# worldfnd/provekit

Hardware: AMD Instinct MI355X
Metric: proofs/sec (noir-r1cs prove hot path, WHIR commit + sumcheck + folding rounds) (higher is better)
Workload: dtype u32x8 (BN254-Fr, 256-bit Montgomery integers); 1 GPU; poseidon-rounds size class: m=21, m_0=20, satisfiable synthetic R1CS (786429 constraints, 1048571 witnesses, a constant term in half of the rows of A and B), batch-2 WHIR commit + zk-sumcheck + 4-round WHIR opening, queries [109, 28, 16, 11]/9, pow_bits [19.0, 16.0, 16.0, 18.0]/11.0 (WhirConfig::new derivation, security 128, ConjectureList), blinding WHIR n=8 queries [122]/31, Skyscraper-sponge tr; launcher=single process

## Files before the change

provekit_amd/csrc/ntt.hip:

```cpp
#include <algorithm>
#include <map>
#include <mutex>
#include <vector>

#include <atomic>

#define PK_BASE_PRIO 1
#include "internal.hpp"
#include "ntt_regs.hpp"

using namespace pk;

namespace {

constexpr int BT = 4;
constexpr int NTHREADS = 256;

__device__ __forceinline__ fe root28_mont() {
    fe r;
    r.v[0] = 0x725b19f0u; r.v[1] = 0x9bd61b6eu; r.v[2] = 0x41112ed4u; r.v[3] = 0x402d111eu;
    r.v[4] = 0x8ef62abcu; r.v[5] = 0x00e0a7ebu; r.v[6] = 0xa58a7e85u; r.v[7] = 0x2a3c09f0u;
    return fe_to_montx(r);
}

__global__ void twiddle_init_kernel(fe* W, unsigned log_n) {
    if (threadIdx.x == 0 && blockIdx.x == 0) {
        fe_store(W, fe_one());
        fe w = root28_mont();
        for (unsigned i = log_n; i < 28; i++) w = fe_sqrx(w);
        if (log_n > 0) fe_store(W + 1, w);
    }
}
__global__ __launch_bounds__(256) void twiddle_double_kernel(fe* W, size_t h) {
    size_t j = (size_t)blockIdx.x * blockDim.x + threadIdx.x;
    if (j >= h) return;
    fe wh = fe_load(W + h);
    if (j == 0) return;
    fe_store(W + h + j, fe_mulx(fe_load(W + j), wh));
}
__global__ void twiddle_seed_kernel(fe* W, size_t h) {
    if (threadIdx.x == 0 && blockIdx.x == 0) fe_store(W + h, fe_sqrx(fe_load(W + h / 2)));
}

__global__ __launch_bounds__(256) void twiddle_scale_kernel(const fe* __restrict__ W, fe* __restrict__ Ws, size_t n) {
    size_t j = (size_t)blockIdx.x * blockDim.x + threadIdx.x;
    if (j >= n) return;
    fe c = fe_zero();
    c.v[0] = 32u;
    fe_store(Ws + j, fe_mulx(fe_load(W + j), c));
}

__global__ __launch_bounds__(256) void twiddle_shoup_kernel(const fe* __restrict__ X, u32* __restrict__ T, size_t n) {
    size_t j = (size_t)blockIdx.x * blockDim.x + threadIdx.x;
    if (j >= n) return;
    const fe29 c = unpack29<0>(fe_from_montx(fe_load(X + j)));
    const fe29 cq = shoup_quotient29(c);
#pragma unroll
    for (int l = 0; l < 9; l++) T[TW29S_WORDS * j + l] = c.v[l];
#pragma unroll
    for (int l = 0; l < 9; l++) T[TW29S_WORDS * j + 9 + l] = cq.v[l];
}

__global__ __launch_bounds__(256) void twiddle_pass_table_kernel(const u32* __restrict__ src, u32* __restrict__ T, size_t rows_k, size_t row, size_t mul,
                                                                 size_t mask) {
    const size_t i = (size_t)blockIdx.x * blockDim.x + threadIdx.x;
    if (i >= rows_k * row) return;
    const size_t k = i / row, v = i % row;
    const u32* q = src + TW29S_WORDS * ((mul * k * v) & mask);
#pragma unroll
    for (int l = 0; l < TW29S_WORDS; l++) T[TW29S_WORDS * i + l] = q[l];
}

struct PassParams {
    const fe* in;
    fe* out;
    size_t in_col_stride, out_col_stride;
    size_t in_stride_r, in_stride_v, in_stride_u;
    size_t out_stride_r, out_stride_v, out_stride_u;
    unsigned log_v;
    size_t nonzero;
    size_t in_nat_r, in_nat_v, in_nat_u;
    const fe* W;
    const fe* Wtw;
    const u32* W29;
    const u32* Wtw29;
    const u32* Tpass29;
    size_t tp_row;
    size_t tiles;
    unsigned ncols;
    int xcd_tiles;
    int lazy_store;
    size_t n_mask;
    size_t tw_mul;
    size_t wr_step;
    const fe* in_poly[16];
    unsigned in_fold;
    int pre_terms;
    size_t pre_stride, pre_elem, pre_ku, pre_kv;
    const u32* Wpre29;
};

template <int LOG_R, bool IN_R_CONTIG>
__global__ __launch_bounds__(NTHREADS) void ntt_pass_kernel(PassParams p) {
    PK_LATENCY_PRIO();
    constexpr int R = 1 << LOG_R;
    constexpr int TILE = R * BT;
    extern __shared__ uint4 lds[];
    uint4* lo = lds;
    uint4* hi = lds + TILE;
    uint4* wlo = lds + 2 * TILE;
    uint4* whi = wlo + (R / 2 > 0 ? R / 2 : 1);

    const unsigned tid = threadIdx.x;
    const size_t tile = blockIdx.x;
    const size_t vblocks = ((size_t)1 << p.log_v) / BT;
    const size_t u = tile / vblocks, vb = tile % vblocks;
    const size_t v0 = vb * BT;
    const size_t col = blockIdx.y;
    const fe* in = p.in + col * p.in_col_stride + u * p.in_stride_u + v0 * p.in_stride_v;
    fe* out = p.out + col * p.out_col_stride + u * p.out_stride_u + v0 * p.out_stride_v;
    const size_t nat0 = u * p.in_nat_u + v0 * p.in_nat_v;

    for (int j = tid; j < R / 2; j += NTHREADS) {
        const uint4* q = reinterpret_cast<const uint4*>(p.W + (size_t)j * p.wr_step);
        wlo[j] = q[0];
        whi[j] = q[1];
    }
    for (int e = tid; e < TILE; e += NTHREADS) {
        int r, b;
        if (IN_R_CONTIG) {
            r = e % R;
            b = e / R;
        } else {
            b = e % BT;
            r = e / BT;
        }
        size_t nat = nat0 + (size_t)r * p.in_nat_r + (size_t)b * p.in_nat_v;
        uint4 a0 = make_uint4(0, 0, 0, 0), a1 = a0;
        if (nat < p.nonzero) {
            const uint4* q = reinterpret_cast<const uint4*>(in + (size_t)r * p.in_stride_r + (size_t)b * p.in_stride_v);
            a0 = q[0];
            a1 = q[1];
        }
        lo[r * BT + b] = a0;
        hi[r * BT + b] = a1;
    }
    __syncthreads();

#pragma unroll 1
    for (int s = 0; s < LOG_R; s++) {
        const int half = R >> (s + 1);
        for (int t = tid; t < (R / 2) * BT; t += NTHREADS) {
            int b = t % BT, j = t / BT;
            int pos = j & (half - 1);
            int i0 = ((j - pos) << 1) + pos;
            int i1 = i0 + half;
            int a0i = i0 * BT + b, a1i = i1 * BT + b;
            fe x0, x1;
            {
                uint4 l0 = lo[a0i], h0 = hi[a0i], l1 = lo[a1i], h1 = hi[a1i];
                x0.v[0] = l0.x; x0.v[1] = l0.y; x0.v[2] = l0.z; x0.v[3] = l0.w;
                x0.v[4] = h0.x; x0.v[5] = h0.y; x0.v[6] = h0.z; x0.v[7] = h0.w;
                x1.v[0] = l1.x; x1.v[1] = l1.y; x1.v[2] = l1.z; x1.v[3] = l1.w;
                x1.v[4] = h1.x; x1.v[5] = h1.y; x1.v[6] = h1.z; x1.v[7] = h1.w;
            }
            fe sum = fe_add(x0, x1);
            fe dif = fe_sub(x0, x1);
            int widx = pos << s;
            if (widx != 0) {
                uint4 wl = wlo[widx], wh = whi[widx];
                fe w;
                w.v[0] = wl.x; w.v[1] = wl.y; w.v[2] = wl.z; w.v[3] = wl.w;
                w.v[4] = wh.x; w.v[5] = wh.y; w.v[6] = wh.z; w.v[7] = wh.w;
                dif = fe_mulx(dif, w);
            }
            lo[a0i] = make_uint4(sum.v[0], sum.v[1], sum.v[2], sum.v[3]);
            hi[a0i] = make_uint4(sum.v[4], sum.v[5], sum.v[6], sum.v[7]);
            lo[a1i] = make_uint4(dif.v[0], dif.v[1], dif.v[2], dif.v[3]);
            hi[a1i] = make_uint4(dif.v[4], dif.v[5], dif.v[6], dif.v[7]);
        }
        __syncthreads();
    }

    for (int e = tid; e < TILE; e += NTHREADS) {
        int b = e % BT, k = e / BT;
        int r = LOG_R == 0 ? 0 : (int)(__brev((unsigned)k) >> (LOG_R ? 32 - LOG_R : 1));
        uint4 l0 = lo[r * BT + b], h0 = hi[r * BT + b];
        fe x;
        x.v[0] = l0.x; x.v[1] = l0.y; x.v[2] = l0.z; x.v[3] = l0.w;
        x.v[4] = h0.x; x.v[5] = h0.y; x.v[6] = h0.z; x.v[7] = h0.w;
        if (p.tw_mul != 0) {
            size_t ex = (p.tw_mul * (size_t)k * (v0 + b)) & p.n_mask;
            if (ex != 0) x = fe_mulx(x, fe_load(p.W + ex));
        }
        fe_store(out + (size_t)k * p.out_stride_r + (size_t)b * p.out_stride_v, x);
    }
}

__host__ __device__ __forceinline__ constexpr int bitrev_c(int v, int bits) {
    int r = 0;
    for (int i = 0; i < bits; i++) r |= ((v >> i) & 1) << (bits - 1 - i);
    return r;
}

struct Ntt8Ctx {
    const fe* in;
    const fe* cin;
    fe* out;
    size_t nat0, v0, k10;
    unsigned tid;
};

template <int LE, int LOG_R, int J, bool PRE>
__device__ __forceinline__ void ntt8_round(fe29 (&x)[1 << LE], const PassParams& p, const Ntt8Ctx& c, u32* planes) {
    constexpr int NX = 1 << LE;
    constexpr int LOGB = 11 - LOG_R, BTT = 1 << LOGB;
    constexpr int NR = (LOG_R + LE - 1) / LE;
    constexpr int D0 = LOG_R - LE * (NR - 1);
    constexpr int D = J == 0 ? D0 : LE;
    constexpr int DONE = J == 0 ? 0 : D0 + LE * (J - 1);
    constexpr int POS = LOGB + LOG_R - DONE - D;
    constexpr int E = LE - D;
    constexpr int REST = POS - LOGB;
    constexpr int LO = POS - E;
    const unsigned tid = c.tid;
    const int base_idx = (int)((tid & ((1u << LO) - 1)) << E) | (int)((tid >> LO) << (POS + D));
#define PK_TILE_INDEX(reg) (base_idx | ((reg) & ((1 << E) - 1)) | (((reg) >> E) << POS))
    if (J == 0) {
#pragma unroll
        for (int reg = 0; reg < NX; reg++) {
            const int I = PK_TILE_INDEX(reg);
            const int r = I >> LOGB, b = I & (BTT - 1);
            const size_t nat = c.nat0 + (size_t)r * p.in_nat_r + (size_t)b * p.in_nat_v;
            if constexpr (PRE) {
                const size_t k1 = c.k10 + (size_t)b * p.pre_kv;
                x[reg] = pre_load_sum(p.pre_terms, [&](int n1, fe29& y) {
                    const size_t t = nat + (size_t)n1 * p.pre_stride;
                    if (t >= p.nonzero) return false;
                    y = mul_tw(unpack29<0>(fe_load(c.cin + t * p.pre_elem)), tw29s_load(p.Wpre29, (k1 * t) & p.n_mask));
                    return true;
                });
            } else {
                fe t = fe_zero();
                if (nat < p.nonzero) t = fe_load(c.in + (size_t)r * p.in_stride_r + (size_t)b * p.in_stride_v);
                x[reg] = unpack29<0>(t);
            }
        }
    } else {
        __syncthreads();
#pragma unroll
        for (int reg = 0; reg < NX; reg++) {
            const int I = PK_TILE_INDEX(reg);
#pragma unroll
            for (int l = 0; l < 9; l++) x[reg].v[l] = planes[l * 2048 + I];
        }
        __syncthreads();
    }
    dft_regs<LE, D>(x);
    const int m = (base_idx >> LOGB) & ((1 << REST) - 1);
    if (J + 1 < NR) {
        const size_t unit = p.wr_step << (LOG_R - D - REST);
#pragma unroll
        for (int reg = 0; reg < NX; reg++) {
            const int a = bitrev_c(reg >> E, D);
            fe29 y = a == 0 ? red29(x[reg]) : mul_tw(x[reg], tw29s_load(p.W29, (size_t)(a * m) * unit));
            const int I = (PK_TILE_INDEX(reg) & ~(((1 << D) - 1) << POS)) | (a << POS);
#pragma unroll
            for (int l = 0; l < 9; l++) planes[l * 2048 + I] = y.v[l];
        }
    } else {
        const int rr = base_idx >> LOGB;
        int k_hi = 0;
#pragma unroll
        for (int j = 0; j < J; j++) {
            const int dj = j == 0 ? D0 : LE, done_j = j == 0 ? 0 : D0 + LE * (j - 1);
            k_hi |= ((rr >> (LOG_R - done_j - dj)) & ((1 << dj) - 1)) << done_j;
        }
        constexpr int KLO = DONE;
#pragma unroll
        for (int reg = 0; reg < NX; reg++) {
            const int a = bitrev_c(reg >> E, D);
            const int b = PK_TILE_INDEX(reg) & (BTT - 1);
            const int k = k_hi | (a << KLO);
            fe29 y;
            if (p.tw_mul && p.Tpass29) {
                y = mul_tw(x[reg], tw29s_load(p.Tpass29, (size_t)k * p.tp_row + (c.v0 + b)));
            } else if (p.tw_mul) {
                size_t ex = (p.tw_mul * (size_t)k * (c.v0 + b)) & p.n_mask;
                y = mul_tw(x[reg], tw29s_load(p.Wtw29, ex));
            } else {
                y = a == 0 ? red29(x[reg]) : red29w(x[reg]);
            }
            fe_store(c.out + (size_t)k * p.out_stride_r + (size_t)b * p.out_stride_v, p.lazy_store ? pack29(y) : pack_canon29(y));
        }
    }
#undef PK_TILE_INDEX
}

template <int LE, int LOG_R, int J, bool PRE>
__device__ __forceinline__ void ntt8_rounds_from(fe29 (&x)[1 << LE], const PassParams& p, const Ntt8Ctx& c, u32* planes) {
    constexpr int NR = (LOG_R + LE - 1) / LE;
    if constexpr (J < NR) {
        ntt8_round<LE, LOG_R, J, PRE>(x, p, c, planes);
        ntt8_rounds_from<LE, LOG_R, J + 1, PRE>(x, p, c, planes);
    }
}

template <int LE, int LOG_R, bool IN_R_CONTIG, bool PRE>
__global__ __launch_bounds__(2048 >> LE) __attribute__((amdgpu_waves_per_eu(4, 4))) void ntt8_pass_kernel(PassParams p) {
    PK_LATENCY_PRIO();
    constexpr int LOGB = 11 - LOG_R;
    extern __shared__ u32 planes[];
    const size_t vblocks = ((size_t)1 << p.log_v) >> LOGB;
    size_t tile, col;
    if (p.xcd_tiles) {
        const size_t j = blockIdx.x >> 3;
        col = j % p.ncols;
        tile = (j / p.ncols) * 8 + (blockIdx.x & 7);
    } else {
        tile = blockIdx.x % p.tiles;
        col = blockIdx.x / p.tiles;
    }
    const size_t u = tile / vblocks, vb = tile % vblocks;
    Ntt8Ctx c;
    c.v0 = vb << LOGB;
    c.cin = p.in_poly[0] ? p.in_poly[col >> p.in_fold] + (col & (((size_t)1 << p.in_fold) - 1)) : p.in + col * p.in_col_stride;
    c.in = c.cin + u * p.in_stride_u + c.v0 * p.in_stride_v;
    c.k10 = u * p.pre_ku + c.v0 * p.pre_kv;
    c.out = p.out + col * p.out_col_stride + u * p.out_stride_u + c.v0 * p.out_stride_v;
    c.nat0 = u * p.in_nat_u + c.v0 * p.in_nat_v;
    c.tid = threadIdx.x;
    fe29 x[1 << LE];
    ntt8_rounds_from<LE, LOG_R, 0, PRE>(x, p, c, planes);
}

template <int FW_MAX>
__global__ __launch_bounds__(256) void deinterleave_kernel(const fe* __restrict__ c, fe* __restrict__ S, size_t L, unsigned fw,
                                                           size_t col_stride) {
    PK_LATENCY_PRIO();
    extern __shared__ uint4 tl[];
    const unsigned TT = 1024 / fw;
    size_t t0 = (size_t)blockIdx.x * TT;
    const fe* src = c + t0 * fw;
    for (unsigned e = threadIdx.x; e < 1024; e += 256) {
        size_t t = t0 + e / fw;
        uint4 a0 = make_uint4(0, 0, 0, 0), a1 = a0;
        if (t < L) {
            const uint4* q = reinterpret_cast<const uint4*>(src + e);
            a0 = q[0];
            a1 = q[1];
        }
        tl[2 * e] = a0;
        tl[2 * e + 1] = a1;
    }
    __syncthreads();
    for (unsigned e = threadIdx.x; e < 1024; e += 256) {
        unsigned j = e / TT, tt = e % TT;
        size_t t = t0 + tt;
        if (t < L) {
            unsigned src_e = tt * fw + j;
            uint4* q = reinterpret_cast<uint4*>(S + (size_t)j * col_stride + t);
            q[0] = tl[2 * src_e];
            q[1] = tl[2 * src_e + 1];
        }
    }
}

__global__ __launch_bounds__(256) void ntt_shard_prestep_kernel(const fe* __restrict__ S, size_t s_col_stride, size_t L, fe* __restrict__ Y,
                                                                size_t y_col_stride, size_t Ng , unsigned g, unsigned G,
                                                                const fe* __restrict__ W , size_t n_mask) {
    PK_LATENCY_PRIO();
    const size_t col = blockIdx.y;
    const fe* x = S + col * s_col_stride;
    fe* y = Y + col * y_col_stride;
    const size_t stride = (size_t)gridDim.x * blockDim.x;
    for (size_t n = (size_t)blockIdx.x * blockDim.x + threadIdx.x; n < Ng; n += stride) {
        fe acc = fe_zero();
        for (unsigned s = 0; s < G; s++) {
            size_t idx = n + (size_t)s * Ng;
            if (idx >= L) break;
            fe v = fe_load(x + idx);
            size_t e = ((size_t)((s * g) % G) * Ng) & n_mask;
            if (e) v = fe_mulx(v, fe_load(W + e));
            acc = fe_add(acc, v);
        }
        size_t e = (n * (size_t)g) & n_mask;
        if (e) acc = fe_mulx(acc, fe_load(W + e));
        fe_store(y + n, acc);
    }
}

struct TableStore {
    std::mutex mu;
    std::map<unsigned long long, void*> tables;
    unsigned contexts = 0;
};
TableStore& store_of(int device) {
    static std::mutex mu;
    static std::map<int, TableStore> stores;
    std::lock_guard<std::mutex> lock(mu);
    return stores[device];
}
enum TableKind : unsigned long long { TK_W = 1, TK_WS = 2, TK_W29 = 3, TK_WS29 = 4, TK_PASS = 5 };
template <class T, class Fill>
int table(pk_ctx* ctx, TableKind kind, unsigned key, size_t bytes, const T** out, Fill fill) {
    const unsigned long long id = (kind << 56) | key;
    auto it = ctx->tables.find(id);
    if (it == ctx->tables.end()) {
        TableStore& S = store_of(ctx->device);
        std::lock_guard<std::mutex> lock(S.mu);
        auto st = S.tables.find(id);
        if (st == S.tables.end()) {
            T* made = nullptr;
            PK_HIP(ctx, hipMalloc((void**)&made, bytes));
            fill(made);
            PK_LAUNCH_CHECK(ctx);
            PK_WAIT(ctx);
            st = S.tables.emplace(id, (void*)made).first;
        }
        it = ctx->tables.emplace(id, st->second).first;
    }
    *out = (const T*)it->second;
    return PK_OK;
}

int get_twiddles(pk_ctx* ctx, unsigned log_n, const fe** out) {
    const size_t n = (size_t)1 << log_n;
    return table(ctx, TK_W, log_n, 32 * std::max<size_t>(n, 2), out, [&](fe* W) {
        twiddle_init_kernel<<<1, 64, 0, ctx->stream>>>(W, log_n);
        for (size_t h = 2; h < n; h <<= 1) {
            twiddle_seed_kernel<<<1, 64, 0, ctx->stream>>>(W, h);
            unsigned grid = (unsigned)((h + 255) / 256);
            twiddle_double_kernel<<<grid, 256, 0, ctx->stream>>>(W, h);
        }
    });
}

struct Twiddles {
    const fe *W, *Ws;
    const u32 *W29, *Ws29;
};
int get_tables(pk_ctx* ctx, unsigned log_n, bool scaled, Twiddles* t) {
    const size_t n = (size_t)1 << log_n, entries = std::max<size_t>(n, 2);
    const unsigned grid = (unsigned)((n + 255) / 256);
    *t = Twiddles{};
    int rc = get_twiddles(ctx, log_n, &t->W);
    t->Ws = t->W;
    if (!rc && scaled)
        rc = table(ctx, TK_WS, log_n, 32 * entries, &t->Ws, [&](fe* Ws) { twiddle_scale_kernel<<<grid, 256, 0, ctx->stream>>>(t->W, Ws, n); });
    if (rc || log_n < 3) return rc;
    auto shoup = [&](TableKind kind, const fe* X, const u32** out) {
        return table(ctx, kind, log_n, 4 * TW29S_WORDS * entries, out, [&](u32* U) { twiddle_shoup_kernel<<<grid, 256, 0, ctx->stream>>>(X, U, n); });
    };
    rc = shoup(TK_W29, t->W, &t->W29);
    t->Ws29 = t->W29;
    if (!rc && scaled) rc = shoup(TK_WS29, t->Ws, &t->Ws29);
    return rc;
}

inline bool pass_is_fast(unsigned log_r, unsigned log_v, size_t N) { return log_r >= 3 && log_v < 62 && log_v >= 11 - log_r && N >= 8; }

constexpr int NTT_LE = 2;

int set_lds_once(pk_ctx* ctx, const void* kernel, size_t lds_bytes, std::atomic<unsigned long long>& done) {
    const unsigned long long dev_bit = 1ull << (ctx->device & 63);
    if (!(done.load(std::memory_order_acquire) & dev_bit)) {
        PK_HIP(ctx, hipFuncSetAttribute(kernel, hipFuncAttributeMaxDynamicSharedMemorySize, (int)lds_bytes));
        done.fetch_or(dev_bit, std::memory_order_release);
    }
    return PK_OK;
}

template <int LE, int LOG_R, bool CONTIG, bool PRE>
int launch_fast(pk_ctx* ctx, const PassParams& pp, unsigned grid) {
    const size_t lds_bytes = 9 * 2048 * 4;
    static std::atomic<unsigned long long> lds_set{0};
    if (int rc = set_lds_once(ctx, (const void*)ntt8_pass_kernel<LE, LOG_R, CONTIG, PRE>, lds_bytes, lds_set)) return rc;
    ntt8_pass_kernel<LE, LOG_R, CONTIG, PRE><<<dim3(grid, 1), 2048 >> LE, lds_bytes, ctx->stream>>>(pp);
    PK_LAUNCH_CHECK(ctx);
    return PK_OK;
}

template <int LOG_R, bool CONTIG>
int launch_lds(pk_ctx* ctx, const PassParams& p, dim3 grid) {
    constexpr int R = 1 << LOG_R;
    const size_t lds_bytes = (size_t)(2 * R * BT + 2 * (R / 2 > 0 ? R / 2 : 1)) * 16;
    static std::atomic<unsigned long long> lds_set{0};
    if (int rc = set_lds_once(ctx, (const void*)ntt_pass_kernel<LOG_R, CONTIG>, lds_bytes, lds_set)) return rc;
    ntt_pass_kernel<LOG_R, CONTIG><<<grid, NTHREADS, lds_bytes, ctx->stream>>>(p);
    PK_LAUNCH_CHECK(ctx);
    return PK_OK;
}

template <int LOG_R>
int launch_pass_r(pk_ctx* ctx, const PassParams& p, bool in_r_contig, size_t tiles, unsigned ncols) {
    if (pass_is_fast(LOG_R, p.log_v, p.n_mask + 1)) {
        ProfScope prof(ctx, in_r_contig ? "ntt_pass_last" : "ntt_pass");
        const size_t tiles8 = (tiles * BT) >> (11 - LOG_R);
        PassParams pp = p;
        pp.tiles = tiles8;
        pp.ncols = ncols;
        pp.xcd_tiles = ((p.Tpass29 != nullptr || p.in_poly[0] != nullptr) && tiles8 % 8 == 0) ? 1 : 0;
        PK_REQUIRE(ctx, tiles8 * ncols < ((size_t)1 << 31), "NTT launch too large");
        const unsigned grid = (unsigned)(tiles8 * ncols);
        constexpr int LR = LOG_R >= 3 ? LOG_R : 3;
        if (p.pre_terms)
            return in_r_contig ? launch_fast<NTT_LE, LR, true, true>(ctx, pp, grid) : launch_fast<NTT_LE, LR, false, true>(ctx, pp, grid);
        return in_r_contig ? launch_fast<NTT_LE, LR, true, false>(ctx, pp, grid) : launch_fast<NTT_LE, LR, false, false>(ctx, pp, grid);
    }
    PK_REQUIRE(ctx, p.in_poly[0] == nullptr && p.pre_terms == 0, "fused NTT input needs the register-radix pass");
    ProfScope prof(ctx, in_r_contig ? "ntt_pass_last" : "ntt_pass");
    const dim3 grid((unsigned)tiles, ncols);
    return in_r_contig ? launch_lds<LOG_R, true>(ctx, p, grid) : launch_lds<LOG_R, false>(ctx, p, grid);
}

int launch_pass(pk_ctx* ctx, unsigned log_r, const PassParams& p, bool in_r_contig, size_t tiles, unsigned ncols) {
    switch (log_r) {
        case 0: return launch_pass_r<0>(ctx, p, in_r_contig, tiles, ncols);
        case 1: return launch_pass_r<1>(ctx, p, in_r_contig, tiles, ncols);
        case 2: return launch_pass_r<2>(ctx, p, in_r_contig, tiles, ncols);
        case 3: return launch_pass_r<3>(ctx, p, in_r_contig, tiles, ncols);
        case 4: return launch_pass_r<4>(ctx, p, in_r_contig, tiles, ncols);
        case 5: return launch_pass_r<5>(ctx, p, in_r_contig, tiles, ncols);
        case 6: return launch_pass_r<6>(ctx, p, in_r_contig, tiles, ncols);
        case 7: return launch_pass_r<7>(ctx, p, in_r_contig, tiles, ncols);
        case 8: return launch_pass_r<8>(ctx, p, in_r_contig, tiles, ncols);
        case 9: return launch_pass_r<9>(ctx, p, in_r_contig, tiles, ncols);
    }
    return set_err(ctx, PK_ERR_BAD_ARG, "unsupported radix 2^%u", log_r);
}

}

namespace pk {

void ntt_retain_ctx(pk_ctx* ctx) {
    TableStore& S = store_of(ctx->device);
    std::lock_guard<std::mutex> lock(S.mu);
    S.contexts++;
}
void ntt_release_ctx(pk_ctx* ctx) {
    ctx->tables.clear();
    TableStore& S = store_of(ctx->device);
    std::lock_guard<std::mutex> lock(S.mu);
    if (S.contexts && --S.contexts == 0) {
        for (auto& kv : S.tables) (void)hipFree(kv.second);
        S.tables.clear();
    }
}

constexpr size_t PRE_MAX_TERMS = 3;
static_assert(PRE_MAX_TERMS <= 4, "pre_load_sum: red29 takes a sum of at most four products");

struct NttPlan {
    unsigned P;
    unsigned l[3];
    unsigned log_v[3];
    bool fast[3];
    size_t L1;
    bool pre;
};
NttPlan ntt_plan(unsigned log_n, size_t nonzero) {
    NttPlan q{};
    const size_t N = (size_t)1 << log_n;
    q.P = log_n <= 18 ? 2 : 3;
    unsigned left = log_n;
    for (unsigned i = 0; i < q.P; i++) {
        q.l[i] = (left + q.P - i - 1) / (q.P - i);
        left -= q.l[i];
        q.log_v[i] = i + 1 < q.P ? left : q.l[0];
        q.fast[i] = pass_is_fast(q.l[i], q.log_v[i], N);
    }
    const size_t stride1 = N >> q.l[0];
    q.L1 = std::max<size_t>(1, (std::min(nonzero, N) + stride1 - 1) / stride1);
    q.pre = q.L1 <= PRE_MAX_TERMS && q.fast[1];
    return q;
}

bool ntt_scaled_available(unsigned log_n) {
    if (log_n <= 9 || log_n > 27) return false;
    const NttPlan q = ntt_plan(log_n, 0);
    return q.fast[q.P - 2];
}

bool ntt_reads_polys(unsigned log_n, size_t nonzero) {
    if (log_n <= 9) return false;
    const NttPlan q = ntt_plan(log_n, nonzero);
    return q.pre || q.fast[0];
}

struct NttInput {
    const fe* in;
    size_t col_stride;
    const fe* const* polys;
    unsigned fold, npolys;
};

struct NttRun {
    NttPlan plan;
    unsigned log_n;
    bool scaled_out;
    Twiddles tw;
    NttInput src;
    size_t nonzero;
    size_t e;
    fe* scratch;
    fe* out;
    size_t out_col_stride;
};

constexpr unsigned PASS_TABLE_MIN_LOG_N = 19;

static int pass_params(pk_ctx* ctx, const NttRun& t, unsigned i, PassParams* out) {
    const NttPlan& q = t.plan;
    const bool last = i + 1 == q.P;
    const size_t N = (size_t)1 << t.log_n, R1 = (size_t)1 << q.l[0], S1 = N / R1;
    unsigned done = 0;
    for (unsigned j = 0; j < i; j++) done += q.l[j];
    const size_t K = (size_t)1 << done, R = (size_t)1 << q.l[i], S = N / (K * R);
    auto tw29 = [&](unsigned j) { return j + 2 == q.P ? t.tw.Ws29 : t.tw.W29; };
    PassParams p{};
    p.W = t.tw.W;
    p.W29 = t.tw.W29;
    p.Wtw = i + 2 == q.P ? t.tw.Ws : t.tw.W;
    p.Wtw29 = tw29(i);
    p.n_mask = N - 1;
    p.log_v = q.log_v[i];
    p.wr_step = N >> q.l[i];
    if (!last) {
        p.out = t.scratch;
        p.out_col_stride = N;
        p.out_stride_r = S;
        p.out_stride_v = 1;
        p.out_stride_u = i ? R * S : 0;
        p.tw_mul = K;
        p.tp_row = S;
        p.lazy_store = q.fast[i + 1];
    } else {
        p.out = t.out;
        p.out_col_stride = t.out_col_stride;
        p.out_stride_r = K;
        p.out_stride_v = 1;
        p.out_stride_u = q.P == 3 ? R1 : 0;
        p.lazy_store = t.scaled_out;
    }
    if (i == 0 || (i == 1 && q.pre)) {
        p.in = t.src.in;
        p.in_col_stride = t.src.col_stride;
        if (t.src.polys) {
            for (unsigned b = 0; b < t.src.npolys; b++) p.in_poly[b] = t.src.polys[b];
            p.in_fold = t.src.fold;
        }
        p.nonzero = t.nonzero;
        p.in_nat_r = S;
        p.in_nat_v = last ? 0 : 1;
        if (i == 0) {
            p.in_stride_r = S * t.e;
            p.in_stride_v = t.e;
        } else {
            p.pre_terms = (int)q.L1;
            p.pre_stride = S1;
            p.pre_elem = t.e;
            p.pre_ku = last ? 0 : 1;
            p.pre_kv = last ? 1 : 0;
            p.Wpre29 = tw29(0);
        }
    } else {
        p.in = t.scratch;
        p.in_col_stride = N;
        p.nonzero = 1;
        p.in_stride_r = last ? 1 : S;
        p.in_stride_v = last ? S1 : 1;
        p.in_stride_u = last ? (q.P == 3 ? R : 0) : R * S;
    }
    if (!last && t.log_n >= PASS_TABLE_MIN_LOG_N && q.fast[i]) {
        const unsigned key = t.log_n | ((i + 1) << 8) | ((t.scaled_out && i + 2 == q.P ? 1u : 0u) << 12);
        const u32* src = p.Wtw29;
        int rc = table(ctx, TK_PASS, key, 4 * TW29S_WORDS * R * S, &p.Tpass29, [&](u32* T) {
            twiddle_pass_table_kernel<<<(unsigned)((R * S + 255) / 256), 256, 0, ctx->stream>>>(src, T, R, S, K, N - 1);
        });
        if (rc) return rc;
    }
    *out = p;
    return PK_OK;
}

int ntt_columns_in(pk_ctx* ctx, const NttInput& src, size_t nonzero, fe* out, size_t out_col_stride, fe* scratch, unsigned log_n,
                   unsigned ncols, bool scaled_out) {
    PK_REQUIRE(ctx, log_n <= 27, "NTT size above 2^27");
    PK_REQUIRE(ctx, !scaled_out || ntt_scaled_available(log_n), "hash-ready NTT output is not available at this size");
    const size_t N = (size_t)1 << log_n;
    Twiddles tw;
    int rc = get_tables(ctx, log_n, scaled_out, &tw);
    if (rc) return rc;
    if (log_n <= 9) {
        PK_REQUIRE(ctx, src.polys == nullptr, "fused NTT input needs more than 512 rows");
        PassParams p{};
        p.in = src.in;
        p.out = out;
        p.in_stride_r = 1;
        p.in_stride_v = src.col_stride;
        p.out_stride_r = 1;
        p.out_stride_v = out_col_stride;
        p.in_nat_r = 1;
        p.nonzero = nonzero;
        p.W = p.Wtw = tw.W;
        p.W29 = p.Wtw29 = tw.W29;
        p.n_mask = N - 1;
        p.wr_step = 1;
        p.log_v = 62;
        unsigned full = ncols / BT, rem = ncols % BT;
        if (full && (rc = launch_pass(ctx, log_n, p, true, full, 1))) return rc;
        for (unsigned c = ncols - rem; c < ncols; c++) {
            PassParams q = p;
            q.in = src.in + (size_t)c * src.col_stride;
            q.out = out + (size_t)c * out_col_stride;
            q.in_stride_v = 0;
            q.out_stride_v = 0;
            if ((rc = launch_pass(ctx, log_n, q, true, 1, 1))) return rc;
        }
        return PK_OK;
    }
    PK_REQUIRE(ctx, scratch != nullptr, "scratch required for N > 512");
    NttRun t{ntt_plan(log_n, nonzero), log_n, scaled_out, tw, src, nonzero, 1, scratch, out, out_col_stride};
    if (src.polys) {
        PK_REQUIRE(ctx, t.plan.pre || t.plan.fast[0], "fused NTT input needs the register-radix pass");
        PK_REQUIRE(ctx, src.npolys >= 1 && src.npolys <= 16 && ((size_t)src.npolys << src.fold) == ncols, "bad fused NTT input");
        t.e = (size_t)1 << src.fold;
    }
    for (unsigned i = t.plan.pre ? 1 : 0; i < t.plan.P; i++) {
        PassParams p;
        if ((rc = pass_params(ctx, t, i, &p)) || (rc = launch_pass(ctx, t.plan.l[i], p, i + 1 == t.plan.P, (N >> t.plan.l[i]) / BT, ncols)))
            return rc;
    }
    return PK_OK;
}

int ntt_columns(pk_ctx* ctx, const fe* in, size_t in_col_stride, size_t nonzero, fe* out, size_t out_col_stride, fe* scratch,
                unsigned log_n, unsigned ncols, bool scaled_out) {
    const NttInput src{in, in_col_stride, nullptr, 0, 0};
    return ntt_columns_in(ctx, src, nonzero, out, out_col_stride, scratch, log_n, ncols, scaled_out);
}

int deinterleave(pk_ctx* ctx, const fe* coeffs, size_t n_coeffs, unsigned fold, fe* S, size_t col_stride) {
    size_t fw = (size_t)1 << fold;
    size_t L = n_coeffs / fw;
    PK_REQUIRE(ctx, fw <= 1024, "fold too large");
    size_t TT = 1024 / fw;
    ProfScope prof(ctx, "deinterleave");
    unsigned grid = (unsigned)((L + TT - 1) / TT);
    deinterleave_kernel<1024><<<grid, 256, 1024 * 32, ctx->stream>>>(coeffs, S, L, (unsigned)fw, col_stride);
    PK_LAUNCH_CHECK(ctx);
    return PK_OK;
}

static int check_encode_args(pk_ctx* ctx, const uint64_t* const* d_coeffs, unsigned batch, unsigned n_vars, unsigned log_inv_rate,
                             unsigned fold, const uint64_t* d_leaves, const uint64_t* d_scratch) {
    PK_REQUIRE(ctx, d_coeffs && d_leaves && d_scratch, "null pointer");
    PK_REQUIRE(ctx, batch >= 1 && batch <= 16, "batch out of range");
    PK_REQUIRE(ctx, fold <= n_vars && fold <= 8, "fold out of range");
    PK_REQUIRE(ctx, n_vars + log_inv_rate >= fold && n_vars + log_inv_rate - fold <= 27, "domain too large (two-adicity 28)");
    return PK_OK;
}

int rs_encode_x(pk_ctx* ctx, const uint64_t* const* d_coeffs, unsigned batch, unsigned n_vars, unsigned log_inv_rate, unsigned fold,
                uint64_t* d_leaves, uint64_t* d_scratch, bool scaled) {
    if (int rc = check_encode_args(ctx, d_coeffs, batch, n_vars, log_inv_rate, fold, d_leaves, d_scratch)) return rc;
    unsigned log_rows = n_vars + log_inv_rate - fold;
    size_t rows = (size_t)1 << log_rows, fw = (size_t)1 << fold;
    size_t L = ((size_t)1 << n_vars) / fw;
    for (unsigned b = 0; b < batch; b++) PK_REQUIRE(ctx, d_coeffs[b], "null polynomial pointer");
    fe* S = (fe*)d_scratch;
    fe* S2 = S + (size_t)batch * fw * rows;
    if (ntt_reads_polys(log_rows, L)) {
        const NttInput src{nullptr, 0, (const fe* const*)d_coeffs, fold, batch};
        return ntt_columns_in(ctx, src, L, (fe*)d_leaves, rows, S, log_rows, (unsigned)(batch * fw), scaled);
    }
    for (unsigned b = 0; b < batch; b++) {
        int rc = pk::deinterleave(ctx, (const fe*)d_coeffs[b], (size_t)1 << n_vars, fold, S + (size_t)b * fw * rows, rows);
        if (rc) return rc;
    }
    return pk::ntt_columns(ctx, S, rows, L, (fe*)d_leaves, rows, S2, log_rows, (unsigned)(batch * fw), scaled);
}

int rs_encode_shard_x(pk_ctx* ctx, const uint64_t* const* d_coeffs, unsigned batch, unsigned n_vars, unsigned log_inv_rate, unsigned fold,
                      unsigned shard, unsigned n_shards, uint64_t* d_leaves_local, uint64_t* d_scratch, bool scaled) {
    if (int rc = check_encode_args(ctx, d_coeffs, batch, n_vars, log_inv_rate, fold, d_leaves_local, d_scratch)) return rc;
    PK_REQUIRE(ctx, is_pow2(n_shards) && shard < n_shards, "n_shards must be a power of two and shard < n_shards");
    const unsigned log_rows = n_vars + log_inv_rate - fold, log_g = ilog2(n_shards);
    PK_REQUIRE(ctx, log_g <= log_rows, "more shards than leaves");
    if (n_shards == 1) return rs_encode_x(ctx, d_coeffs, batch, n_vars, log_inv_rate, fold, d_leaves_local, d_scratch, scaled);
    const size_t rows = (size_t)1 << log_rows, fw = (size_t)1 << fold, Ng = rows >> log_g;
    const size_t L = ((size_t)1 << n_vars) / fw;
    const unsigned ncols = (unsigned)(batch * fw);
    fe* S = (fe*)d_scratch;
    fe* Y = S + (size_t)ncols * rows;
    fe* S2 = Y + (size_t)ncols * Ng;
    for (unsigned b = 0; b < batch; b++) {
        PK_REQUIRE(ctx, d_coeffs[b], "null polynomial pointer");
        int rc = pk::deinterleave(ctx, (const fe*)d_coeffs[b], (size_t)1 << n_vars, fold, S + (size_t)b * fw * rows, rows);
        if (rc) return rc;
    }
    const fe* W = nullptr;
    int rc = get_twiddles(ctx, log_rows, &W);
    if (rc) return rc;
    {
        ProfScope prof(ctx, "ntt_shard_prestep");
        dim3 grid((unsigned)std::min<size_t>((Ng + 255) / 256, 1024), ncols);
        ntt_shard_prestep_kernel<<<grid, 256, 0, ctx->stream>>>(S, rows, L, Y, Ng, Ng, shard, n_shards, W, rows - 1);
    }
    PK_LAUNCH_CHECK(ctx);
    return pk::ntt_columns(ctx, Y, Ng, Ng, (fe*)d_leaves_local, Ng, S2, log_rows - log_g, ncols, scaled);
}
}

extern "C" {

int pk_ntt(pk_ctx* ctx, const uint64_t* d_in, uint64_t* d_out, unsigned log_n, unsigned ncols) {
    PK_ENTER(ctx);
    PK_REQUIRE(ctx, d_in && d_out, "null pointer");
    PK_REQUIRE(ctx, ncols >= 1, "ncols must be >= 1");
    size_t N = (size_t)1 << log_n;
    fe* scratch = nullptr;
    if (log_n > 9) PK_HIP(ctx, hipMalloc((void**)&scratch, 32 * N * ncols));
    int rc = pk::ntt_columns(ctx, (const fe*)d_in, N, N, (fe*)d_out, N, scratch, log_n, ncols, false);
    if (scratch) {
        hipError_t e = wait_ctx(ctx);
        (void)hipFree(scratch);
        if (!rc && e != hipSuccess) rc = set_err(ctx, PK_ERR_HIP, "ntt failed: %s", hipGetErrorString(e));
    }
    return rc;
}

int pk_rs_encode(pk_ctx* ctx, const uint64_t* const* d_coeffs, unsigned batch, unsigned n_vars, unsigned log_inv_rate,
                 unsigned fold, uint64_t* d_leaves, uint64_t* d_scratch) {
    PK_ENTER(ctx);
    return pk::rs_encode_x(ctx, d_coeffs, batch, n_vars, log_inv_rate, fold, d_leaves, d_scratch, false);
}

int pk_rs_encode_shard(pk_ctx* ctx, const uint64_t* const* d_coeffs, unsigned batch, unsigned n_vars, unsigned log_inv_rate,
                       unsigned fold, unsigned shard, unsigned n_shards, uint64_t* d_leaves_local, uint64_t* d_scratch) {
    PK_ENTER(ctx);
    return pk::rs_encode_shard_x(ctx, d_coeffs, batch, n_vars, log_inv_rate, fold, shard, n_shards, d_leaves_local, d_scratch, false);
}

}
```

Before: 282.3 proofs/s.

## Make NTT workgroups persistent across columns and prefetch next tile via global_load_lds

The fast NTT pass now launches roughly two workgroups per CU and has each loop over a group of columns instead of one workgroup per (tile, column). While a column's final round stores its results, the next column's input tile is loaded asynchronously into LDS with global_load_lds, so the load latency overlaps compute and stores. This cuts launch and scheduling overhead and hides input latency. The cost is fewer resident waves, manual waitcnt handling that could be fragile, and an env-var override for the residency target.

After: 276.7 proofs/s. -2.0%, worse.

```diff
diff --git a/provekit_amd/csrc/ntt.hip b/provekit_amd/csrc/ntt.hip
--- a/provekit_amd/csrc/ntt.hip
+++ b/provekit_amd/csrc/ntt.hip
@@ -1,4 +1,5 @@
 #include <algorithm>
+#include <cstdlib>
 #include <map>
 #include <mutex>
 #include <vector>
@@ -88,6 +89,7 @@
     size_t tp_row;
     size_t tiles;
     unsigned ncols;
+    unsigned col_groups, group_cols;
     int xcd_tiles;
     int lazy_store;
     size_t n_mask;
@@ -204,47 +206,93 @@
 }
 
 struct Ntt8Ctx {
-    const fe* in;
     const fe* cin;
     fe* out;
     size_t nat0, v0, k10;
     unsigned tid;
 };
 
+template <int LE, int LOG_R, int J>
+struct Ntt8Geom {
+    static constexpr int NX = 1 << LE;
+    static constexpr int LOGB = 11 - LOG_R, BTT = 1 << LOGB;
+    static constexpr int NR = (LOG_R + LE - 1) / LE;
+    static constexpr int D0 = LOG_R - LE * (NR - 1);
+    static constexpr int D = J == 0 ? D0 : LE;
+    static constexpr int DONE = J == 0 ? 0 : D0 + LE * (J - 1);
+    static constexpr int POS = LOGB + LOG_R - DONE - D;
+    static constexpr int E = LE - D;
+    static constexpr int REST = POS - LOGB;
+    static constexpr int LO = POS - E;
+    static __device__ __forceinline__ int base(unsigned tid) { return (int)((tid & ((1u << LO) - 1)) << E) | (int)((tid >> LO) << (POS + D)); }
+    static __device__ __forceinline__ int index(int base_idx, int reg) { return base_idx | (reg & ((1 << E) - 1)) | ((reg >> E) << POS); }
+};
+
+typedef __attribute__((address_space(3))) void* lds_void_ptr;
+typedef const __attribute__((address_space(1))) void* global_void_ptr;
+template <int LE, int LOG_R>
+__device__ __forceinline__ void ntt8_fetch_tile(const PassParams& p, Ntt8Ctx& c, const fe* in, u32* planes) {
+    using G = Ntt8Geom<LE, LOG_R, 0>;
+    asm volatile("" : "+v"(c.tid));
+    const int base_idx = G::base(c.tid);
+    const unsigned wave = __builtin_amdgcn_readfirstlane(c.tid >> 6);
+#pragma unroll
+    for (int reg = 0; reg < G::NX; reg++) {
+        const int I = G::index(base_idx, reg);
+        const int r = I >> G::LOGB, b = I & (G::BTT - 1);
+        const size_t nat = c.nat0 + (size_t)r * p.in_nat_r + (size_t)b * p.in_nat_v;
+        if (nat < p.nonzero) {
+            const char* q = reinterpret_cast<const char*>(in + (size_t)r * p.in_stride_r + (size_t)b * p.in_stride_v);
+#pragma unroll
+            for (int h = 0; h < 2; h++)
+                __builtin_amdgcn_global_load_lds((global_void_ptr)(q + 16 * h), (lds_void_ptr)(planes + 256 * ((wave * G::NX + reg) * 2 + h)), 16, 0, 0);
+        }
+    }
+}
+template <int LE, int LOG_R>
+__device__ __forceinline__ void ntt8_take_tile(fe29 (&x)[1 << LE], const PassParams& p, const Ntt8Ctx& c, const u32* planes) {
+    using G = Ntt8Geom<LE, LOG_R, 0>;
+    const int base_idx = G::base(c.tid);
+    const uint4* image = reinterpret_cast<const uint4*>(planes) + (size_t)(c.tid >> 6) * (G::NX * 2 * 64) + (c.tid & 63);
+    __builtin_amdgcn_s_waitcnt(0x0F70);
+#pragma unroll
+    for (int reg = 0; reg < G::NX; reg++) {
+        const int I = G::index(base_idx, reg);
+        const int r = I >> G::LOGB, b = I & (G::BTT - 1);
+        const size_t nat = c.nat0 + (size_t)r * p.in_nat_r + (size_t)b * p.in_nat_v;
+        fe t = fe_zero();
+        if (nat < p.nonzero) {
+            const uint4 lo = image[(reg * 2) * 64], hi = image[(reg * 2 + 1) * 64];
+            t.v[0] = lo.x; t.v[1] = lo.y; t.v[2] = lo.z; t.v[3] = lo.w;
+            t.v[4] = hi.x; t.v[5] = hi.y; t.v[6] = hi.z; t.v[7] = hi.w;
+        }
+        x[reg] = unpack29<0>(t);
+    }
+    __syncthreads();
+}
+
 template <int LE, int LOG_R, int J, bool PRE>
-__device__ __forceinline__ void ntt8_round(fe29 (&x)[1 << LE], const PassParams& p, const Ntt8Ctx& c, u32* planes) {
-    constexpr int NX = 1 << LE;
-    constexpr int LOGB = 11 - LOG_R, BTT = 1 << LOGB;
-    constexpr int NR = (LOG_R + LE - 1) / LE;
-    constexpr int D0 = LOG_R - LE * (NR - 1);
-    constexpr int D = J == 0 ? D0 : LE;
-    constexpr int DONE = J == 0 ? 0 : D0 + LE * (J - 1);
-    constexpr int POS = LOGB + LOG_R - DONE - D;
-    constexpr int E = LE - D;
-    constexpr int REST = POS - LOGB;
-    constexpr int LO = POS - E;
-    const unsigned tid = c.tid;
-    const int base_idx = (int)((tid & ((1u << LO) - 1)) << E) | (int)((tid >> LO) << (POS + D));
-#define PK_TILE_INDEX(reg) (base_idx | ((reg) & ((1 << E) - 1)) | (((reg) >> E) << POS))
-    if (J == 0) {
+__device__ __forceinline__ void ntt8_round(fe29 (&x)[1 << LE], const PassParams& p, Ntt8Ctx& c, const fe* next_in, u32* planes) {
+    using G = Ntt8Geom<LE, LOG_R, J>;
+    constexpr int NX = G::NX, LOGB = G::LOGB, BTT = G::BTT, NR = G::NR, D0 = G::D0, D = G::D, DONE = G::DONE, POS = G::POS, E = G::E, REST = G::REST;
+    asm volatile("" : "+v"(c.tid));
+    const int base_idx = G::base(c.tid);
+#define PK_TILE_INDEX(reg) G::index(base_idx, reg)
+    if constexpr (J == 0 && !PRE) {
+        ntt8_take_tile<LE, LOG_R>(x, p, c, planes);
+    } else if constexpr (J == 0) {
 #pragma unroll
         for (int reg = 0; reg < NX; reg++) {
             const int I = PK_TILE_INDEX(reg);
             const int r = I >> LOGB, b = I & (BTT - 1);
             const size_t nat = c.nat0 + (size_t)r * p.in_nat_r + (size_t)b * p.in_nat_v;
-            if constexpr (PRE) {
-                const size_t k1 = c.k10 + (size_t)b * p.pre_kv;
-                x[reg] = pre_load_sum(p.pre_terms, [&](int n1, fe29& y) {
-                    const size_t t = nat + (size_t)n1 * p.pre_stride;
-                    if (t >= p.nonzero) return false;
-                    y = mul_tw(unpack29<0>(fe_load(c.cin + t * p.pre_elem)), tw29s_load(p.Wpre29, (k1 * t) & p.n_mask));
-                    return true;
-                });
-            } else {
-                fe t = fe_zero();
-                if (nat < p.nonzero) t = fe_load(c.in + (size_t)r * p.in_stride_r + (size_t)b * p.in_stride_v);
-                x[reg] = unpack29<0>(t);
-            }
+            const size_t k1 = c.k10 + (size_t)b * p.pre_kv;
+            x[reg] = pre_load_sum(p.pre_terms, [&](int n1, fe29& y) {
+                const size_t t = nat + (size_t)n1 * p.pre_stride;
+                if (t >= p.nonzero) return false;
+                y = mul_tw(unpack29<0>(fe_load(c.cin + t * p.pre_elem)), tw29s_load(p.Wpre29, (k1 * t) & p.n_mask));
+                return true;
+            });
         }
     } else {
         __syncthreads();
@@ -277,17 +325,26 @@
             k_hi |= ((rr >> (LOG_R - done_j - dj)) & ((1 << dj) - 1)) << done_j;
         }
         constexpr int KLO = DONE;
+        const bool fetch = !PRE && next_in != nullptr;
+        if (fetch && !p.tw_mul) ntt8_fetch_tile<LE, LOG_R>(p, c, next_in, planes);
 #pragma unroll
         for (int reg = 0; reg < NX; reg++) {
             const int a = bitrev_c(reg >> E, D);
             const int b = PK_TILE_INDEX(reg) & (BTT - 1);
             const int k = k_hi | (a << KLO);
             fe29 y;
+            const auto fetch_behind = [&](const tw29s& t) {
+                if (reg == NX - 1 && fetch) {
+                    __builtin_amdgcn_s_waitcnt(0x0F70);
+                    ntt8_fetch_tile<LE, LOG_R>(p, c, next_in, planes);
+                }
+                return t;
+            };
             if (p.tw_mul && p.Tpass29) {
-                y = mul_tw(x[reg], tw29s_load(p.Tpass29, (size_t)k * p.tp_row + (c.v0 + b)));
+                y = mul_tw(x[reg], fetch_behind(tw29s_load(p.Tpass29, (size_t)k * p.tp_row + (c.v0 + b))));
             } else if (p.tw_mul) {
                 size_t ex = (p.tw_mul * (size_t)k * (c.v0 + b)) & p.n_mask;
-                y = mul_tw(x[reg], tw29s_load(p.Wtw29, ex));
+                y = mul_tw(x[reg], fetch_behind(tw29s_load(p.Wtw29, ex)));
             } else {
                 y = a == 0 ? red29(x[reg]) : red29w(x[reg]);
             }
@@ -298,11 +355,11 @@
 }
 
 template <int LE, int LOG_R, int J, bool PRE>
-__device__ __forceinline__ void ntt8_rounds_from(fe29 (&x)[1 << LE], const PassParams& p, const Ntt8Ctx& c, u32* planes) {
+__device__ __forceinline__ void ntt8_rounds_from(fe29 (&x)[1 << LE], const PassParams& p, Ntt8Ctx& c, const fe* next_in, u32* planes) {
     constexpr int NR = (LOG_R + LE - 1) / LE;
     if constexpr (J < NR) {
-        ntt8_round<LE, LOG_R, J, PRE>(x, p, c, planes);
-        ntt8_rounds_from<LE, LOG_R, J + 1, PRE>(x, p, c, planes);
+        ntt8_round<LE, LOG_R, J, PRE>(x, p, c, next_in, planes);
+        ntt8_rounds_from<LE, LOG_R, J + 1, PRE>(x, p, c, next_in, planes);
     }
 }
 
@@ -312,26 +369,35 @@
     constexpr int LOGB = 11 - LOG_R;
     extern __shared__ u32 planes[];
     const size_t vblocks = ((size_t)1 << p.log_v) >> LOGB;
-    size_t tile, col;
+    size_t tile, grp;
     if (p.xcd_tiles) {
         const size_t j = blockIdx.x >> 3;
-        col = j % p.ncols;
-        tile = (j / p.ncols) * 8 + (blockIdx.x & 7);
+        grp = j % p.col_groups;
+        tile = (j / p.col_groups) * 8 + (blockIdx.x & 7);
     } else {
         tile = blockIdx.x % p.tiles;
-        col = blockIdx.x / p.tiles;
+        grp = blockIdx.x / p.tiles;
     }
     const size_t u = tile / vblocks, vb = tile % vblocks;
     Ntt8Ctx c;
     c.v0 = vb << LOGB;
-    c.cin = p.in_poly[0] ? p.in_poly[col >> p.in_fold] + (col & (((size_t)1 << p.in_fold) - 1)) : p.in + col * p.in_col_stride;
-    c.in = c.cin + u * p.in_stride_u + c.v0 * p.in_stride_v;
     c.k10 = u * p.pre_ku + c.v0 * p.pre_kv;
-    c.out = p.out + col * p.out_col_stride + u * p.out_stride_u + c.v0 * p.out_stride_v;
     c.nat0 = u * p.in_nat_u + c.v0 * p.in_nat_v;
     c.tid = threadIdx.x;
-    fe29 x[1 << LE];
-    ntt8_rounds_from<LE, LOG_R, 0, PRE>(x, p, c, planes);
+    const size_t tile_in = u * p.in_stride_u + c.v0 * p.in_stride_v, tile_out = u * p.out_stride_u + c.v0 * p.out_stride_v;
+    const auto column = [&](size_t col) {
+        return p.in_poly[0] ? p.in_poly[col >> p.in_fold] + (col & (((size_t)1 << p.in_fold) - 1)) : p.in + col * p.in_col_stride;
+    };
+    const size_t col0 = grp * p.group_cols, col1 = col0 + p.group_cols < p.ncols ? col0 + p.group_cols : p.ncols;
+    if constexpr (!PRE) ntt8_fetch_tile<LE, LOG_R>(p, c, column(col0) + tile_in, planes);
+#pragma unroll 1
+    for (size_t col = col0; col < col1; col++) {
+        c.cin = column(col);
+        c.out = p.out + col * p.out_col_stride + tile_out;
+        const fe* next_in = col + 1 < col1 ? column(col + 1) + tile_in : nullptr;
+        fe29 x[1 << LE];
+        ntt8_rounds_from<LE, LOG_R, 0, PRE>(x, p, c, next_in, planes);
+    }
 }
 
 template <int FW_MAX>
@@ -501,8 +567,14 @@
         pp.tiles = tiles8;
         pp.ncols = ncols;
         pp.xcd_tiles = ((p.Tpass29 != nullptr || p.in_poly[0] != nullptr) && tiles8 % 8 == 0) ? 1 : 0;
-        PK_REQUIRE(ctx, tiles8 * ncols < ((size_t)1 << 31), "NTT launch too large");
-        const unsigned grid = (unsigned)(tiles8 * ncols);
+        size_t resident = (size_t)ctx->num_cus * 2;
+        if (const char* e = getenv("PK_NTT_RESIDENT_WGS"))
+            if (const long v = atol(e); v > 0) resident = (size_t)v;
+        const size_t want = std::max<size_t>(1, (resident + tiles8 - 1) / tiles8);
+        pp.group_cols = (unsigned)((ncols + std::min<size_t>(want, ncols) - 1) / std::min<size_t>(want, ncols));
+        pp.col_groups = (ncols + pp.group_cols - 1) / pp.group_cols;
+        PK_REQUIRE(ctx, tiles8 * pp.col_groups < ((size_t)1 << 31), "NTT launch too large");
+        const unsigned grid = (unsigned)(tiles8 * pp.col_groups);
         constexpr int LR = LOG_R >= 3 ? LOG_R : 3;
         if (p.pre_terms)
             return in_r_contig ? launch_fast<NTT_LE, LR, true, true>(ctx, pp, grid) : launch_fast<NTT_LE, LR, false, true>(ctx, pp, grid);
```
